# PASSIONLab/BELLA

Measured on AMD Instinct MI355X. Metric: candidate overlap pairs/sec, higher is better.
Workload: dtype u16/u32 integer

## Files before the change

### bella_amd/csrc/order.hpp

```cpp
#pragma once
#include <hip/hip_runtime.h>
#include <stdint.h>
#include "../../include/bella_hip.h"
#include "core.hpp"
#include "slotorder.hpp"
#include "util.hpp"

namespace bella {

constexpr uint32_t kOrderWaveHt = 1024;
constexpr uint32_t kOrderLdsHt = 16384;
constexpr uint32_t kOrderBlock = 256;
constexpr uint32_t kOrderBigGrid = 512;
constexpr uint32_t kOrderOneLaunchMax = 32768;
constexpr uint64_t kOrderWsBytes = (uint64_t)6 * 65536;

struct OrderArgs {
    const uint64_t* flopptr;
    const uint64_t* colptrC;
    const uint32_t* nnzC;
    const uint32_t* flops;
    uint32_t nreads, i0, stride, nown;
    const bella_pair* tmp_pairs;
    const bella_pair_ext* tmp_ext;
    bella_pair* pairs;
    bella_pair_ext* ext;
    uint64_t* totals;
    uint32_t* nbig;
    uint32_t* biglist;
    uint8_t* ws;
};

__device__ __forceinline__ void order_copy_record(const OrderArgs& a, uint64_t from, uint64_t to, uint32_t cid) {
    uint4 rec = *(const uint4*)(a.tmp_pairs + from);
    asm volatile("" : "+v"(rec.y));
    rec.y = cid;
    *(uint4*)(a.pairs + to) = rec;
    if (a.ext) a.ext[to] = a.tmp_ext[from];
}

__device__ __forceinline__ bool wave_next_free(const uint32_t* T2, uint16_t* nf, uint32_t ht) {
    const uint32_t lane = lane_id();
    const uint32_t nb = (ht + 63u) >> 6;
    uint32_t carry = 0xFFFFFFFFu;
#pragma unroll 1
    for (int sweep = 0; sweep < 2; ++sweep) {
        for (uint32_t b = nb; b-- > 0;) {
            const uint32_t s = (b << 6) + lane;
            const bool empty = s < ht && T2[s] == kEmpty;
            const unsigned long long m = __ballot(empty);
            if (sweep == 1 && s < ht) {
                const unsigned long long up = m >> lane;
                nf[s] = (uint16_t)(up ? s + (uint32_t)__ffsll((long long)up) - 1u : carry);
            }
            if (m) carry = (b << 6) + (uint32_t)__ffsll((long long)m) - 1u;
        }
        if (carry == 0xFFFFFFFFu) return false;
    }
    return true;
}
__device__ __forceinline__ void wave_rank_slots(const uint32_t* T2, uint16_t* ord, uint32_t ht) {
    const uint32_t lane = lane_id();
    const uint32_t nb = (ht + 63u) >> 6;
    uint32_t base = 0;
    for (uint32_t b = 0; b < nb; ++b) {
        const uint32_t s = (b << 6) + lane;
        const uint32_t it = s < ht ? T2[s] : kEmpty;
        const unsigned long long m = __ballot(it != kEmpty);
        if (it != kEmpty) ord[base + (uint32_t)__popcll(m & ((1ull << lane) - 1ull))] = (uint16_t)(it & 0xFFFFu);
        base += (uint32_t)__popcll(m);
    }
}

template <uint32_t HT, uint32_t HTLO>
__global__ __launch_bounds__(kOrderBlock) void k_order_wave(OrderArgs a) {
    __shared__ uint32_t s_T2[kOrderBlock / 64][HT];
    __shared__ uint16_t s_ord[kOrderBlock / 64][HT];
    const uint32_t j0 = blockIdx.x * (kOrderBlock / 64) + wave_id();
    const uint32_t lane = lane_id();
    if (HTLO == 0 && j0 == 0 && lane == 0) a.totals[0] = a.colptrC[a.nreads];
    if (j0 >= a.nown) return;
    const uint32_t i = a.i0 + j0 * a.stride;
    uint32_t nz = a.nnzC[i];
    uint64_t src = a.flopptr[i], dst = a.colptrC[i];
    uint32_t tmax = a.flops[i];
    asm volatile("" : "+v"(nz), "+v"(src), "+v"(dst), "+v"(tmax));
    const uint32_t d = nz & ~kOrderedBit;
    if (!d) return;
    if (nz & kOrderedBit) {
        if (HTLO == 0) for (uint32_t r = lane; r < d; r += 64) order_copy_record(a, src + r, dst + r, i);
        return;
    }
    const uint32_t ht = pow2_at_least(16u, d);
    if (ht > kOrderWaveHt) {
        if (HTLO == 0 && lane == 0) a.biglist[atomicAdd(a.nbig, 1u)] = i;
        return;
    }
    if (ht > HT || ht <= HTLO) return;
    uint32_t* T2 = s_T2[wave_id()];
    uint16_t* ord = s_ord[wave_id()];
    for (uint32_t s = lane; s < ht; s += 64) T2[s] = kEmpty;
    constexpr uint32_t NI = HT / 64;
    uint32_t key[NI], fp[NI];
#pragma unroll
    for (uint32_t u = 0; u < NI; ++u) {
        const uint32_t j = lane + 64 * u;
        key[u] = 0; fp[u] = 0xFFFFFFFFu;
        if (j < d) { const uint2 kf = *(const uint2*)(a.tmp_pairs + src + j); key[u] = kf.x; fp[u] = kf.y; }
    }
    group_sync<64>();
    uint32_t prev = 0;
    for (uint32_t rd = 0;; ++rd) {
        const uint32_t bound = round_bound(rd, ht, d, tmax);
        if (rd) { (void)wave_next_free(T2, ord, ht); group_sync<64>(); }
#pragma unroll
        for (uint32_t u = 0; u < NI; ++u) {
            if (fp[u] < prev || fp[u] >= bound) continue;
            const uint32_t home = (key[u] * 107u) & (ht - 1), item = (fp[u] << 16) | (lane + 64 * u);
            if (rd) slot_insert<true>(T2, ord, ht - 1, home, item);
            else slot_insert<false>(T2, ord, ht - 1, home, item);
        }
        group_sync<64>();
        if (bound >= tmax) break;
        prev = bound;
    }
    wave_rank_slots(T2, ord, ht);
    group_sync<64>();
    {
        uint32_t r = lane;
        for (; r + 192 < d; r += 256) {
            uint4 rec[4];
#pragma unroll
            for (uint32_t u = 0; u < 4; ++u) rec[u] = *(const uint4*)(a.tmp_pairs + src + ord[r + 64 * u]);
#pragma unroll
            for (uint32_t u = 0; u < 4; ++u) { asm volatile("" : "+v"(rec[u].y)); rec[u].y = i; *(uint4*)(a.pairs + dst + r + 64 * u) = rec[u]; }
            if (a.ext) {
#pragma unroll
                for (uint32_t u = 0; u < 4; ++u) a.ext[dst + r + 64 * u] = a.tmp_ext[src + ord[r + 64 * u]];
            }
        }
        for (; r < d; r += 64) order_copy_record(a, src + ord[r], dst + r, i);
    }
}

__global__ __launch_bounds__(kOrderBlock) void k_order_block(OrderArgs a) {
    extern __shared__ __attribute__((aligned(16))) uint8_t smem[];
    __shared__ uint32_t scr[16];
    const uint32_t nbig = *a.nbig;
    const uint32_t tid = threadIdx.x;
    for (uint32_t x = blockIdx.x; x < nbig; x += gridDim.x) {
        const uint32_t i = a.biglist[x];
        const uint32_t d = a.nnzC[i] & ~kOrderedBit;
        const uint64_t src = a.flopptr[i], dst = a.colptrC[i];
        const uint32_t ht = pow2_at_least(16u, d);
        uint32_t* T2;
        uint16_t* ord;
        if (ht <= kOrderLdsHt) { T2 = (uint32_t*)smem; ord = (uint16_t*)(smem + (size_t)4 * kOrderLdsHt); }
        else { uint8_t* w = a.ws + (uint64_t)blockIdx.x * kOrderWsBytes; T2 = (uint32_t*)w; ord = (uint16_t*)(w + (size_t)4 * 65536); }
        for (uint32_t s = tid; s < ht; s += kOrderBlock) T2[s] = kEmpty;
        __syncthreads();
        const uint32_t tmax = a.flops[i];
        uint32_t prev = 0;
        for (uint32_t rd = 0;; ++rd) {
            const uint32_t bound = round_bound(rd, ht, d, tmax);
            if (rd) { (void)build_next_free<(int)kOrderBlock>(T2, ord, ht, scr); __syncthreads(); }
            for (uint32_t j = tid; j < d; j += kOrderBlock) {
                const uint2 kf = *(const uint2*)(a.tmp_pairs + src + j);
                if (kf.y < prev || kf.y >= bound) continue;
                const uint32_t home = (kf.x * 107u) & (ht - 1), item = (kf.y << 16) | j;
                if (rd) slot_insert<true>(T2, ord, ht - 1, home, item);
                else slot_insert<false>(T2, ord, ht - 1, home, item);
            }
            __syncthreads();
            if (bound >= tmax) break;
            prev = bound;
        }
        {
            const uint32_t c = (ht + kOrderBlock - 1) / kOrderBlock;
            const uint32_t lo = tid * c < ht ? tid * c : ht, hi = lo + c < ht ? lo + c : ht;
            uint32_t occ = 0;
            for (uint32_t s = lo; s < hi; ++s) occ += T2[s] != kEmpty ? 1u : 0u;
            uint32_t tot;
            uint32_t rank = block_excl_scan<kOrderBlock / 64>(occ, scr, &tot);
            for (uint32_t s = lo; s < hi; ++s) {
                const uint32_t it = T2[s];
                if (it != kEmpty) ord[rank++] = (uint16_t)(it & 0xFFFFu);
            }
        }
        __syncthreads();
        for (uint32_t r = tid; r < d; r += kOrderBlock) order_copy_record(a, src + ord[r], dst + r, i);
        __syncthreads();
    }
}

}
```

Before: 12.76 billion.

## Keep full records in registers and scatter via LDS staging for coalesced writes

The wave-level ordering kernel now loads each full 16-byte record into registers once, instead of loading only key and fingerprint and later re-gathering whole records from global memory by sorted index. The ranking pass inverts the mapping so each record learns its output rank. Records are then scattered into an LDS staging buffer (reusing the hash table) in chunks and written out contiguously. This removes the second random global gather at the cost of extra LDS traffic, syncs and register pressure. Per-column scalars are also made wave-uniform via readfirstlane.

```diff
diff --git a/bella_amd/csrc/order.hpp b/bella_amd/csrc/order.hpp
--- a/bella_amd/csrc/order.hpp
+++ b/bella_amd/csrc/order.hpp
@@ -59,7 +59,7 @@
     }
     return true;
 }
-__device__ __forceinline__ void wave_rank_slots(const uint32_t* T2, uint16_t* ord, uint32_t ht) {
+__device__ __forceinline__ void wave_rank_records(const uint32_t* T2, uint16_t* rk, uint32_t ht) {
     const uint32_t lane = lane_id();
     const uint32_t nb = (ht + 63u) >> 6;
     uint32_t base = 0;
@@ -67,14 +67,14 @@
         const uint32_t s = (b << 6) + lane;
         const uint32_t it = s < ht ? T2[s] : kEmpty;
         const unsigned long long m = __ballot(it != kEmpty);
-        if (it != kEmpty) ord[base + (uint32_t)__popcll(m & ((1ull << lane) - 1ull))] = (uint16_t)(it & 0xFFFFu);
+        if (it != kEmpty) rk[it & 0xFFFFu] = (uint16_t)(base + (uint32_t)__popcll(m & ((1ull << lane) - 1ull)));
         base += (uint32_t)__popcll(m);
     }
 }
 
 template <uint32_t HT, uint32_t HTLO>
 __global__ __launch_bounds__(kOrderBlock) void k_order_wave(OrderArgs a) {
-    __shared__ uint32_t s_T2[kOrderBlock / 64][HT];
+    __shared__ __attribute__((aligned(16))) uint32_t s_T2[kOrderBlock / 64][HT];
     __shared__ uint16_t s_ord[kOrderBlock / 64][HT];
     const uint32_t j0 = blockIdx.x * (kOrderBlock / 64) + wave_id();
     const uint32_t lane = lane_id();
@@ -85,7 +85,10 @@
     uint64_t src = a.flopptr[i], dst = a.colptrC[i];
     uint32_t tmax = a.flops[i];
     asm volatile("" : "+v"(nz), "+v"(src), "+v"(dst), "+v"(tmax));
-    const uint32_t d = nz & ~kOrderedBit;
+    const uint32_t d = __builtin_amdgcn_readfirstlane(nz & ~kOrderedBit);
+    tmax = __builtin_amdgcn_readfirstlane(tmax);
+    src = ((uint64_t)__builtin_amdgcn_readfirstlane((uint32_t)(src >> 32)) << 32) | __builtin_amdgcn_readfirstlane((uint32_t)src);
+    dst = ((uint64_t)__builtin_amdgcn_readfirstlane((uint32_t)(dst >> 32)) << 32) | __builtin_amdgcn_readfirstlane((uint32_t)dst);
     if (!d) return;
     if (nz & kOrderedBit) {
         if (HTLO == 0) for (uint32_t r = lane; r < d; r += 64) order_copy_record(a, src + r, dst + r, i);
@@ -101,12 +104,13 @@
     uint16_t* ord = s_ord[wave_id()];
     for (uint32_t s = lane; s < ht; s += 64) T2[s] = kEmpty;
     constexpr uint32_t NI = HT / 64;
-    uint32_t key[NI], fp[NI];
+    uint4 rec[NI];
+    constexpr uint32_t kNoRank = 0xFFFFFFFFu;
 #pragma unroll
     for (uint32_t u = 0; u < NI; ++u) {
         const uint32_t j = lane + 64 * u;
-        key[u] = 0; fp[u] = 0xFFFFFFFFu;
-        if (j < d) { const uint2 kf = *(const uint2*)(a.tmp_pairs + src + j); key[u] = kf.x; fp[u] = kf.y; }
+        rec[u] = *(const uint4*)(a.tmp_pairs + src + (j < d ? j : d - 1));
+        if (j >= d) rec[u].y = kNoRank;
     }
     group_sync<64>();
     uint32_t prev = 0;
@@ -115,8 +119,9 @@
         if (rd) { (void)wave_next_free(T2, ord, ht); group_sync<64>(); }
 #pragma unroll
         for (uint32_t u = 0; u < NI; ++u) {
-            if (fp[u] < prev || fp[u] >= bound) continue;
-            const uint32_t home = (key[u] * 107u) & (ht - 1), item = (fp[u] << 16) | (lane + 64 * u);
+            asm volatile("" : "+v"(rec[u].x), "+v"(rec[u].y));
+            if (rec[u].y < prev || rec[u].y >= bound) continue;
+            const uint32_t home = (rec[u].x * 107u) & (ht - 1), item = (rec[u].y << 16) | (lane + 64 * u);
             if (rd) slot_insert<true>(T2, ord, ht - 1, home, item);
             else slot_insert<false>(T2, ord, ht - 1, home, item);
         }
@@ -124,22 +129,39 @@
         if (bound >= tmax) break;
         prev = bound;
     }
-    wave_rank_slots(T2, ord, ht);
+    wave_rank_records(T2, ord, ht);
     group_sync<64>();
-    {
-        uint32_t r = lane;
-        for (; r + 192 < d; r += 256) {
-            uint4 rec[4];
-#pragma unroll
-            for (uint32_t u = 0; u < 4; ++u) rec[u] = *(const uint4*)(a.tmp_pairs + src + ord[r + 64 * u]);
-#pragma unroll
-            for (uint32_t u = 0; u < 4; ++u) { asm volatile("" : "+v"(rec[u].y)); rec[u].y = i; *(uint4*)(a.pairs + dst + r + 64 * u) = rec[u]; }
-            if (a.ext) {
-#pragma unroll
-                for (uint32_t u = 0; u < 4; ++u) a.ext[dst + r + 64 * u] = a.tmp_ext[src + ord[r + 64 * u]];
-            }
-        }
-        for (; r < d; r += 64) order_copy_record(a, src + ord[r], dst + r, i);
+#pragma unroll
+    for (uint32_t u = 0; u < NI; ++u) {
+        const uint32_t j = lane + 64 * u;
+        const uint32_t r = ord[j];
+        rec[u].y = j < d ? r : kNoRank;
+    }
+    if (a.ext) {
+#pragma unroll
+        for (uint32_t u = 0; u < NI; ++u) {
+            const uint32_t j = lane + 64 * u;
+            if (j < d) a.ext[dst + rec[u].y] = a.tmp_ext[src + j];
+        }
+    }
+    group_sync<64>();
+    constexpr uint32_t W = HT / 4;
+    uint4* stage = (uint4*)T2;
+    for (uint32_t wb = 0; wb < d; wb += W) {
+#pragma unroll
+        for (uint32_t u = 0; u < NI; ++u) {
+            const uint32_t r = rec[u].y - wb;
+            if (r < W) { uint4 o = rec[u]; o.y = i; stage[r] = o; }
+        }
+        group_sync<64>();
+        const uint32_t n = d - wb < W ? d - wb : W;
+        bella_pair* out = a.pairs + dst + wb;
+#pragma unroll
+        for (uint32_t t = 0; t < W / 64; ++t) {
+            const uint32_t x = lane + 64 * t;
+            if (x < n) *(uint4*)(out + x) = stage[x];
+        }
+        group_sync<64>();
     }
 }
 
```

Result: faster. 12.97 billion (median of 6 runs) (+1.6%).
